# zoltanmaric/h264-fer

Hardware: AMD Instinct MI355X
Metric: macroblocks/sec encode (1080p full-search ME) + bit-exact bitstream vs ref (higher is better)
Workload: dtype u8; 1 GPU; 1080p IPPP encode, full-search +-16 ME (BASELINE configs[2]); content=textured, coded_size=1920x1072, streams_per_gpu=256, contexts_per_gpu=1, gop=30, qp=12, window=32, maxdiff=3, parallelism=1 x 256 independent closed-GOP streams

## Files before the change

h264-fer_amd/__init__.py:

```python
from .ferhip import (FerHip, FerHipError, Decoder, LiveDecoder, access_units, DeviceBuffer, Y4MReader, decode_streams, unescape_nal, lib_path,
                     load_library, mb_unit, cavlc_blocks, cavlc_parse_blocks, residual_mbs, RES_WRITE, RES_PARSE, mc_sub_mb_parts, MBU_QT, MBU_DEC4, MBU_DEC16, MBU_DECC, MBU_SKIP, TUNE_RESOLVE_WGS, TUNE_RESOLVE_GROUP, TUNE_SPECULATE, TUNE_OVERLAP_SORT, RC_CQP, RC_ABR, RC_QUALITY, QM_SSE, QM_SSIM,
                     QUALITY_RING, Quality, NAL_SLICE, NAL_IDR, NAL_AUTO, NAL_NONE, AU_PARAM_SETS, AU, frame_nal_blocks, frame_nal_blocks_raw,
                     NAL_UNIT, SPLIT_PREFIX, split_nal_blocks, split_nal_blocks_raw, FMT_I420, FMT_NV12, FMT_YUY2, FMT_UYVY, FMT_BGRA, FMT_RGBA, CSC_BT601, CSC_BT709, Pic, pic_table,
                     AU_AVCC, IN_ANNEXB, IN_AVCC, split_avcc_blocks_raw)
from .synth import gen_frame, gen_frames, crop_to_mb, pad_to_mb
from .shard import gops_of_rank, merge_gop_streams, split_nals
```

h264-fer_amd/csrc/fer_me.hip:

```cpp
#include <stdlib.h>
#include "fer_internal.h"
#include "fer_mvpred.h"

#define INF_M 1000000000

struct WList {
    int m;
    int xy;
};

__device__ __forceinline__ int pack_xy(int x, int y) { return (x & 0xffff) | (y << 16); }
__device__ __forceinline__ int unp_x(int xy) { return (int)(short)(xy & 0xffff); }
__device__ __forceinline__ int unp_y(int xy) { return xy >> 16; }

__device__ __forceinline__ void wl_insert(WList &L, int K, int lane, bool valid, int m, int xy)
{
    int thr = lane_bcast(L.m, K - 1);
    unsigned long long mask = __ballot(valid && m < thr);
    while (mask) {
        int src = __ffsll((long long)mask) - 1;
        mask &= mask - 1;
        int cm = lane_bcast(m, src), cxy = lane_bcast(xy, src);
        int pos = __popcll(__ballot(lane < K && L.m <= cm));
        if (pos < K) {
            int um = FER_DPP(L.m, DPP_WAVE_SHR1), uxy = FER_DPP(L.xy, DPP_WAVE_SHR1);
            if (lane > pos && lane < K) {
                L.m = um;
                L.xy = uxy;
            } else if (lane == pos) {
                L.m = cm;
                L.xy = cxy;
            }
        }
    }
}

#define WAVE_LDS_SYNC()                                    \
    do {                                                   \
        __builtin_amdgcn_fence(__ATOMIC_SEQ_CST, "wavefront"); \
        __builtin_amdgcn_wave_barrier();                   \
    } while (0)
__device__ __forceinline__ int lds_rank64(const unsigned *p, unsigned mine, int n4 = 16)
{
    const uint4 *q = (const uint4 *)p;
    int r = 0;
#pragma unroll 4
    for (int i = 0; i < n4; i++) {
        uint4 k = q[i];
        r += (int)(k.x < mine) + (int)(k.y < mine) + (int)(k.z < mine) + (int)(k.w < mine);
    }
    return r;
}

template <int NB, bool ORDERED, class RAW, class FIN, class ARR>
__device__ __forceinline__ bool select_topk_ex(const int (&v)[NB], int K, int lane, int *sel, WList &L, RAW raw, FIN fin, ARR arr)
{
    unsigned *A = (unsigned *)sel, *B = A + 64;
    int *Ci = sel + 128, *Di = sel + 192;
    const unsigned long long lt = (1ull << lane) - 1ull;
    int lmin = 0x7fffffff, lmax = -1, total = 0;
#pragma unroll
    for (int u = 0; u < NB; u++) {
        total += __popcll(__ballot(v[u] >= 0));
        lmin = (int)min((unsigned)lmin, (unsigned)v[u]);
        lmax = max(lmax, v[u]);
    }
    const int need = min(K, total);
    L.m = INF_M;
    L.xy = 0;
    if (need == 0) return true;
    int c = 65;
    if (!__any(lmax >= (1 << 26))) {
        B[lane] = 0xffffffffu;
        int T0 = 0x7fffffff;
        if (__popcll(__ballot(lmin != 0x7fffffff)) >= need) {
            int lo = 0, hi = (1 << 21) - 1;
            if (__popcll(__ballot(lmin <= hi)) >= need) {
                while (lo < hi) {
                    const int mid = (lo + hi) >> 1;
                    if (__popcll(__ballot(lmin <= mid)) >= need)
                        hi = mid;
                    else
                        lo = mid + 1;
                }
                T0 = lo;
            } else {
                T0 = 1 << 21;
            }
        }
        WAVE_LDS_SYNC();
        if (T0 < (1 << 21) && NB * 64 <= 2048) {
            int nsurv = 0;
#pragma unroll
            for (int u = 0; u < NB; u++) {
                const bool take = (unsigned)v[u] <= (unsigned)T0;
                const unsigned long long mk = __ballot(take);
                if (mk) {
                    const int slot = nsurv + (int)__builtin_amdgcn_mbcnt_hi((uint32_t)(mk >> 32), __builtin_amdgcn_mbcnt_lo((uint32_t)mk, 0u));
                    if (take && slot < 64) {
                        B[slot] = ((unsigned)v[u] << 11) | (unsigned)arr(u);
                        Ci[slot] = raw(u);
                    }
                    nsurv += __popcll(mk);
                }
            }
            WAVE_LDS_SYNC();
            c = nsurv;
        }
    }
    if (c <= 64) {
        WAVE_LDS_SYNC();
        const unsigned mine = B[lane];
        const int mypay = Ci[lane];
        const int rk = lds_rank64(B, mine, (__builtin_amdgcn_readfirstlane(c) + 3) >> 2);
        WAVE_LDS_SYNC();
        if (lane < c && rk < need) {
            A[rk] = mine >> 11;
            Di[rk] = mypay;
        }
        WAVE_LDS_SYNC();
        if (lane < need) {
            L.m = (int)A[lane];
            L.xy = fin(Di[lane]);
        }
        WAVE_LDS_SYNC();
        return true;
    }
    if (!ORDERED) return false;
    int *key = sel, *kxy = sel + 64, *key2 = sel + 128, *kxy2 = sel + 192;
    int lo = wave_min(lmin), hi;
    if (__popcll(__ballot(lmin != 0x7fffffff)) >= need)
        hi = wave_max(lmin != 0x7fffffff ? lmin : -1);
    else
        hi = wave_max(lmax);
    while (lo < hi) {
        int mid = lo + ((hi - lo) >> 1);
        int cnt = 0;
#pragma unroll
        for (int u = 0; u < NB; u++) cnt += __popcll(__ballot(v[u] >= 0 && v[u] <= mid));
        if (cnt >= need)
            hi = mid;
        else
            lo = mid + 1;
    }
    const int T = lo;
    int c_less = 0;
#pragma unroll
    for (int u = 0; u < NB; u++) c_less += __popcll(__ballot(v[u] >= 0 && v[u] < T));
    const int take_eq = need - c_less;
    int nsel = 0, eq_seen = 0;
    WAVE_LDS_SYNC();
#pragma unroll
    for (int u = 0; u < NB; u++) {
        bool ok = v[u] >= 0;
        bool eq = ok && v[u] == T;
        unsigned long long meq = __ballot(eq);
        bool take = (ok && v[u] < T) || (eq && eq_seen + __popcll(meq & lt) < take_eq);
        unsigned long long mt = __ballot(take);
        if (take) {
            int pos = nsel + __popcll(mt & lt);
            key[pos] = v[u];
            kxy[pos] = raw(u);
        }
        nsel += __popcll(mt);
        eq_seen += __popcll(meq);
    }
    WAVE_LDS_SYNC();
    int mk = lane < need ? key[lane] : INF_M, mxy = lane < need ? kxy[lane] : 0;
    int rank = 0;
    for (int i = 0; i < need; i++) {
        int ki = key[i];
        rank += (ki < mk) || (ki == mk && i < lane);
    }
    if (lane < need) {
        key2[rank] = mk;
        kxy2[rank] = mxy;
    }
    WAVE_LDS_SYNC();
    if (lane < need) {
        L.m = key2[lane];
        L.xy = fin(kxy2[lane]);
    }
    WAVE_LDS_SYNC();
    return true;
}
template <int NB, class RAW, class FIN>
__device__ __forceinline__ void select_topk(const int (&v)[NB], int K, int lane, int *sel, WList &L, RAW raw, FIN fin)
{
    select_topk_ex<NB, true>(v, K, lane, sel, L, raw, fin, [&](int u) { return u * 64 + lane; });
}

typedef unsigned short u16x2_t __attribute__((ext_vector_type(2)));
typedef short i16x2_t __attribute__((ext_vector_type(2)));
__device__ __forceinline__ uint32_t pk_sub16(uint32_t a, uint32_t b)
{
    return __builtin_bit_cast(uint32_t, (u16x2_t)(__builtin_bit_cast(u16x2_t, a) - __builtin_bit_cast(u16x2_t, b)));
}
__device__ __forceinline__ uint32_t pk_abs16(uint32_t a)
{
    i16x2_t x = __builtin_bit_cast(i16x2_t, a), z = {0, 0};
    return __builtin_bit_cast(uint32_t, __builtin_elementwise_max(x, (i16x2_t)(z - x)));
}
struct SuPk {
    uint32_t s01, s23, s4;
    uint32_t d01, d23, d4;
    uint32_t s12, s34;
    uint32_t e12, e34;
};
__device__ __forceinline__ SuPk su_pack(const int s[5])
{
    SuPk p;
    p.s01 = (uint32_t)s[0] | ((uint32_t)s[1] << 16);
    p.s23 = (uint32_t)s[2] | ((uint32_t)s[3] << 16);
    p.s4 = (uint32_t)s[4];
    p.d01 = (uint32_t)(s[0] - s[1]) << 16;
    p.d23 = (uint32_t)(s[0] - s[2]) | ((uint32_t)(s[0] - s[3]) << 16);
    p.d4 = (uint32_t)(s[0] - s[4]);
    p.s12 = (uint32_t)s[1] | ((uint32_t)s[2] << 16);
    p.s34 = (uint32_t)s[3] | ((uint32_t)s[4] << 16);
    p.e12 = (uint32_t)(s[0] - s[1]) | ((uint32_t)(s[0] - s[2]) << 16);
    p.e34 = (uint32_t)(s[0] - s[3]) | ((uint32_t)(s[0] - s[4]) << 16);
    return p;
}
__device__ __forceinline__ int feat_dist_w(uint32_t a, uint32_t b, uint32_t c, const SuPk &p)
{
    uint32_t t = __builtin_amdgcn_sad_u16(a, p.s01, 0);
    t = __builtin_amdgcn_sad_u16(b, p.s23, t);
    t = __builtin_amdgcn_sad_u16(c, p.s4, t);
    uint32_t kk = __builtin_amdgcn_perm(a, a, 0x01000100);
    t = __builtin_amdgcn_sad_u16(pk_sub16(kk, a), p.d01, t);
    t = __builtin_amdgcn_sad_u16(pk_sub16(kk, b), p.d23, t);
    t = __builtin_amdgcn_sad_u16(pk_sub16(kk, c) & 0xffffu, p.d4, t);
    return (int)t;
}
__device__ __forceinline__ int feat_dist_rec(const uint16_t *__restrict__ rec, const SuPk &p)
{
    const uint32_t *r = (const uint32_t *)rec;
    return feat_dist_w(r[0], r[1], r[2], p);
}
struct FeatRec {
    uint32_t a, b, c;
};
// ... 254 lines not shown
    su[1] = wave_sum(py > 3 ? 0 : v);
    su[2] = wave_sum(px > 3 ? 0 : v);
    su[3] = wave_sum((py & 3) > 1 ? 0 : v);
    su[4] = wave_sum((px & 3) > 1 ? 0 : v);
    if (lane < 5) d.suma[pidx * 5 + lane] = su[lane];
    if (d.basic) {
        if (lane == 0) {
            d.st3n[pidx] = 0;
            d.v0[pidx] = 0;
        }
        return;
    }
    const SuPk sp = su_pack(su);
    PP_MARK(0)

    WList L;
    L.m = INF_M;
    L.xy = 0;
    const int R = window / 2, n = 2 * R + 1;
    const int r2 = window / 16, n2w = 2 * r2 + 1, nloc = n2w * n2w * 16;
    const uint16_t *F0 = d.feat0 + (size_t)s * 6 * ysz;
    const int wb = (n * n + 63) >> 6;
    if ((WIN == 32 || WIN == 16) && !FER_DBGF(d, 3)) {
        constexpr int WCH = 3;
        constexpr int NN = (WIN ? WIN : 32) + 1;
        constexpr int NBc = WIN ? WIN : 32, RPB = 64 / NBc, NWB = (NN + RPB - 1) / RPB;
        constexpr int LB = LocalGeo<RRL>::NB;
        static_assert(LB <= 7, "ME_SEL_NB leaves room for 7 local batches");
        const int ix = lane % NBc, r0 = lane / NBc;
        const int rx = sx - R + ix;
        const bool xok = rx >= 0 && rx < W;
        const int wx = iabs(ix - R) + 4;
        const uint32_t colo = (uint32_t)iclamp(rx, 0, W - 1) * 12u, rowb = (uint32_t)W * 12u;
        auto fin = [&](int idx) {
            if (idx < wb * 64) return pack_xy((idx / n - R) * 4, (idx % n - R) * 4);
            int c = idx - wb * 64;
            int frac = c & 15, pos = c >> 4;
            return pack_xy((pos / n2w - r2) * 4 + (frac & 3), (pos % n2w - r2) * 4 + (frac >> 2));
        };
        uint32_t k0w[NWB];
#pragma unroll
        for (int b2 = 0; b2 < NWB; b2++) {
            const int ry = iclamp(sy - R + b2 * RPB + r0, 0, H - 1);
            k0w[b2] = *(const uint32_t *)((const char *)F0 + (colo + __umul24((uint32_t)ry, rowb)));
        }
        const uint32_t k0c = feat0_load(F0, W, H, sy - R + min(lane, NN - 1), sx + R).a;
        auto second_group = [&](int half) {
            if (half == 0) local_request<RRL>(ip, W, H, sx - RRL, sy - RRL, lane, ld, 1, 2);
        };
        local_metrics<RRL, decltype(second_group), true>(ip, W, H, sx - r2, sy - r2, sp, lane, (uint32_t *)wide_m, sel_lds, 0, 2, &ld, second_group);
        unsigned lminl = 0xffffffffu;
#pragma unroll
        for (int u = 0; u < LB; u++) lminl = min(lminl, (unsigned)sel_lds[u * 64 + lane]);
        int T = 0x7fffffff;
        if (__popcll(__ballot(lminl < (1u << 21))) >= 33) {
            int lo = 0, hi = (1 << 21) - 1;
            while (lo < hi) {
                const int mid = (lo + hi) >> 1;
                if (__popcll(__ballot(lminl <= (unsigned)mid)) >= 33)
                    hi = mid;
                else
                    lo = mid + 1;
            }
            T = lo;
        }
        int *surv = wide_m;
        int ns = 0;
        const uint32_t s0 = (uint32_t)su[0];
        bool done = false;
        if (T != 0x7fffffff) {
            static_assert((NBc / 2) % RPB == 0 && NN <= 64, "a batch stays on one side of the centre row");
            const int iy_lo = max(0, R - sy), iy_hi = min(NN - 1, H - 1 - (sy - R));
            const unsigned long long rowv = ((2ull << iy_hi) - 1ull) & ~((1ull << iy_lo) - 1ull);
            const unsigned long long colv = wave_ballot(xok);
            constexpr unsigned long long GRP = NBc == 64 ? ~0ull : (1ull << NBc) - 1ull;
            const uint32_t w5lo = 5u * (uint32_t)(wx + R - r0), w5hi = 5u * (uint32_t)(wx - R + r0);
            const int arr0 = ix * NN + r0;
#pragma unroll
            for (int b2 = 0; b2 < NWB; b2++) {
                unsigned long long valid = 0;
#pragma unroll
                for (int j = 0; j < RPB; j++)
                    if ((rowv >> (b2 * RPB + j)) & 1ull) valid |= GRP << (j * NBc);
                valid &= colv;
                const uint32_t w5 = b2 * RPB < R ? w5lo - 5u * (uint32_t)(b2 * RPB) : w5hi + 5u * (uint32_t)(b2 * RPB);
                const uint32_t lb = __umul24(w5, __builtin_amdgcn_sad_u16(k0w[b2] & 0xffffu, s0, 0u));
                const unsigned long long mk = wave_ballot(lb <= (uint32_t)T) & valid;
                if (mk) {
                    const int slot = ns + (int)__builtin_amdgcn_mbcnt_hi((uint32_t)(mk >> 32), __builtin_amdgcn_mbcnt_lo((uint32_t)mk, 0u));
                    if (wave_mask_bit(mk) && slot < 128) surv[slot] = arr0 + b2 * RPB;
                    ns += __popcll(mk);
                }
            }
            {
                const uint32_t lb = __umul24(5u * (uint32_t)(R + 4 + iabs(lane - R)), __builtin_amdgcn_sad_u16(k0c & 0xffffu, s0, 0u));
                const unsigned long long mk = sx + R < W ? wave_ballot(lb <= (uint32_t)T) & rowv : 0ull;
                if (mk) {
                    const int slot = ns + (int)__builtin_amdgcn_mbcnt_hi((uint32_t)(mk >> 32), __builtin_amdgcn_mbcnt_lo((uint32_t)mk, 0u));
                    if (wave_mask_bit(mk) && slot < 128) surv[slot] = (NN - 1) * NN + lane;
                    ns += __popcll(mk);
                }
            }
            WAVE_LDS_SYNC();
            if (ns <= 128) {
                int v[2 + LB], ar[2];
#pragma unroll
                for (int b2 = 0; b2 < 2; b2++) {
                    v[b2] = -1;
                    ar[b2] = 0;
                    if (b2 * 64 < ns) {
                        const int idx = b2 * 64 + lane;
                        const bool on = idx < ns;
                        const int ai = on ? surv[idx] : 0;
                        const int cix = ai / NN, ciy = ai - cix * NN;
                        const FeatRec f = feat0_load(F0, W, H, sy - R + ciy, sx - R + cix);
                        const int m = (int)__umul24((uint32_t)(iabs(cix - R) + iabs(ciy - R) + 4), (uint32_t)feat_dist_w(f.a, f.b, f.c, sp));
                        v[b2] = on ? m : -1;
                        ar[b2] = ai;
                    }
                }
#pragma unroll
                for (int u = 0; u < LB; u++) v[2 + u] = sel_lds[u * 64 + lane];
                WAVE_LDS_SYNC();
                auto arrv = [&](int u) { return u < 2 ? ar[u < 2 ? u : 0] : wb * 64 + (u - 2) * 64 + lane; };
                done = select_topk_ex<2 + LB, false>(v, 33, lane, wide_m + 128, L, arrv, fin, arrv);
            }
        }
        PP_MARK(1)
#ifdef FER_STATS
        if (lane == 0) {
            atomicAdd((unsigned long long *)&d.timing[48], 1ull);
            atomicAdd((unsigned long long *)&d.timing[49], done ? 0ull : 1ull);
            atomicAdd((unsigned long long *)&d.timing[50], (unsigned long long)ns);
            atomicAdd((unsigned long long *)&d.timing[51], T == 0x7fffffff ? 1ull : 0ull);
            atomicAdd((unsigned long long *)&d.timing[52], (unsigned long long)(T == 0x7fffffff ? 0 : T));
        }
#endif
        if (!done) {
            WAVE_LDS_SYNC();
            int vloc[LB];
#pragma unroll
            for (int u = 0; u < LB; u++) vloc[u] = sel_lds[u * 64 + lane];
            WAVE_LDS_SYNC();
            auto wide_load = [&](int iy0, FeatRec (&fr)[WCH]) {
#pragma unroll
                for (int q = 0; q < WCH; q++) {
                    int ry = iclamp(sy - R + iy0 + q * RPB + r0, 0, H - 1);
                    const uint32_t *r = (const uint32_t *)((const char *)F0 + (colo + __umul24((uint32_t)ry, rowb)));
                    fr[q].a = r[0];
                    fr[q].b = r[1];
                    fr[q].c = r[2];
                }
            };
            auto wide_eval = [&](int iy0, const FeatRec (&fr)[WCH]) {
#pragma unroll
                for (int q = 0; q < WCH; q++) {
                    const int iy = iy0 + q * RPB + r0;
                    const int ry = sy - R + iy;
                    const int m = (int)__umul24((uint32_t)(wx + iabs(iy - R)), (uint32_t)feat_dist_w(fr[q].a, fr[q].b, fr[q].c, sp));
                    const int bad = (xok && ry >= 0 && ry < H) ? 0 : -1;
                    wide_m[iy < n ? ix * n + iy : ME_WIDE_LDS - 1] = m | bad;
                }
            };
            {
                constexpr int STEP = RPB * WCH;
                FeatRec fa[WCH], fb[WCH];
                wide_load(0, fa);
                for (int iy0 = 0; iy0 < n; iy0 += 2 * STEP) {
                    if (iy0 + STEP < n) wide_load(iy0 + STEP, fb);
                    wide_eval(iy0, fa);
                    if (iy0 + STEP < n) {
                        if (iy0 + 2 * STEP < n) wide_load(iy0 + 2 * STEP, fa);
                        wide_eval(iy0 + STEP, fb);
                    }
                }
            }
            {
                const int iy = min(lane, n - 1);
// ... 858 lines not shown
                take = take && cls;
            }
            const int m = (r + 4) * D;
            const int side = kk0 > P.su[0] ? 1 : 0;
            const unsigned akey = ((unsigned)j << 21) | ((unsigned)(tx + 280) << 10) | (unsigned)(ty + 280);
            const int xy = pack_xy(tx * 4, ty * 4);
            cl_insert(L, lane, take, m, akey | ((unsigned)side << 20), xy);
            if (__any(take && j == 0)) cl_insert(L, lane, take && j == 0, m, akey | (1u << 20), xy);
            {
                int rr = (int)((1.0f + __fsqrt_rn((float)(2 * (k0 + 64) - 1))) * 0.5f);
                while (2 * rr * (rr - 1) + 1 > k0 + 64) rr--;
                while (2 * (rr + 1) * rr + 1 <= k0 + 64) rr++;
                done_r = rr - 1;
            }
            const int t33 = lane_bcast(L.m, 32);
            if (done_r >= rmax) break;
            if (t33 < INF_M && (long long)(done_r + 1 + 4) * dmin > (long long)t33) break;
        }
    }
    L2.m = L.m;
    L2.xy = L.xy;
}

__device__ __forceinline__ int stage2_list(const FerDev &d, int s, int gx, int gy, int lane, const ResPre &P, int genx, int geny,
                                           int *sel_lds, WList &L2)
{
    const int sx = gx * 8, sy = gy * 8;
    L2.m = INF_M;
    L2.xy = 0;
    if (d.basic || FER_DBGF(d, 32)) return 0;
    const uint32_t cfl = (uint32_t)lane_bcast(P.e2[0].y, 41);
    const bool rewalk = (cfl & 0x40000000u) != 0 && ((cfl >> 16) & 15u) == 0;
    if (P.n2raw > FER_ST2_CAP && d.zero_cnt[s] == 0 && !rewalk) {
        resolve_crowded(d, s, sx, sy, lane, P, genx, geny, L2);
    } else if (P.n2raw > FER_ST2_CAP) {
        const SuPk sp = su_pack(P.su);
        int jx;
        walk_buckets(d, s, P.su, sp, sx, sy, lane, (uint32_t *)sel_lds, 0x7fffffff, jx, [&](bool ok, int rank, int rel, int D, uint32_t, bool) {
            (void)rank;
            int tx = rel >> 16, ty = (int)(short)(rel & 0xffff);
            wl_insert(L2, 33, lane, ok, (iabs(tx - genx) + iabs(ty - geny) + 4) * D, pack_xy(tx * 4, ty * 4));
            return false;
        });
    } else {
        int m2[FER_ST2_CAP / 64];
#pragma unroll
        for (int u = 0; u < FER_ST2_CAP / 64; u++) {
            int cc = u * 64 + lane;
            int tx = P.e2[u].x >> 16, ty = (int)(short)(P.e2[u].x & 0xffff);
            m2[u] = (int)__umul24((uint32_t)(iabs(tx - genx) + iabs(ty - geny) + 4), (uint32_t)P.e2[u].y) | (cc < P.n2 ? 0 : -1);
        }
        auto raw2 = [&](int u) { return P.e2[u].x; };
        auto fin2 = [&](int e) { return pack_xy((e >> 16) * 4, (int)(short)(e & 0xffff) * 4); };
        select_topk<FER_ST2_CAP / 64>(m2, 33, lane, sel_lds, L2, raw2, fin2);
    }
    return __popcll(__ballot(lane < 33 && L2.m < 100000000));
}

template <int WIN>
__device__ __forceinline__ void resolve_stage23(const FerDev &d, int s, int gx, int gy, int lane, const ResPre &P, int mvpx, int mvpy,
                                                int *sel_lds, int &k2, int &xy2, int &k3, int &xy3)
{
    k2 = k3 = 0x7fffffff;
    xy2 = xy3 = 0;
    if (d.basic || FER_DBGF(d, 32)) return;
    WList L2;
    const int cnt2 = stage2_list(d, s, gx, gy, lane, P, mvpx >> 2, mvpy >> 2, sel_lds, L2);
    if (FER_DBGF(d, 256)) L2.xy = pack_xy(lane & 7, lane >> 3);
    int b2, b2xy;
    sad_keys<33>(L2, cnt2, lane, ip_stream(d, s), d.W, d.H, gx * 8, gy * 8, P.sb, mvpx, mvpy, b2, b2xy);
    wave_best(b2, b2xy, k2, xy2);
    int key = 0x7fffffff;
    if (lane < P.n3) key = ((P.c3s + iabs(P.c3x - mvpx) + iabs(P.c3y - mvpy)) << 6) | lane;
    wave_best(key, pack_xy(P.c3x, P.c3y), k3, xy3);
}

__device__ __forceinline__ ResNbr nbr_from_field(const FerDev &d, const int *vf, int gx, int gy, int lane)
{
    ResNbr N;
    nbr_avail(gx, gy, d.mbw * 2, N.vB, N.vC, N.vD, N.vC16);
    N.vA = gx > 0;
    const int xa = gx + (lane == 0 ? 0 : (lane == 1 ? 1 : (lane == 2 ? -1 : (lane == 3 ? 2 : -1)))), ya = lane == 4 ? gy : gy - 1;
    const bool val = lane == 0 ? N.vB : (lane == 1 ? N.vC : (lane == 2 ? N.vD : (lane == 3 ? N.vC16 : (lane == 4 && N.vA))));
    const int w = val ? vf[part_slot(d.mbw, xa, ya)] : 0;
    N.B = lane_bcast(w, 0);
    N.C = lane_bcast(w, 1);
    N.D = lane_bcast(w, 2);
    N.C16 = lane_bcast(w, 3);
    N.A = lane_bcast(w, 4);
    return N;
}

#ifndef SPEC_WAVES
#define SPEC_WAVES 7
#endif
template <int WIN>
__global__ __launch_bounds__(256) __attribute__((amdgpu_waves_per_eu(SPEC_WAVES, SPEC_WAVES))) void k_me_spec(FerDev d)
{
    __shared__ __attribute__((aligned(16))) uint32_t loc_all[4][LocalGeo<2>::HTAB + LocalGeo<2>::NB * 64];
    __shared__ int skipflag;
    static_assert(LocalGeo<2>::HTAB >= 256, "the selection's scratch fits the row sums");
    const int lane = threadIdx.x & 63;
    const int part = __builtin_amdgcn_readfirstlane(threadIdx.x >> 6);
    const int s = blockIdx.y;
    if (d.hdr[s * 4 + 3] != 0) return;
    const int mb = (int)xcd_swizzle(blockIdx.x, gridDim.x);
    const int mbx = mb % d.mbw, mby = mb / d.mbw;
// ... 260 lines not shown
        d.timing[7] = gw;
    }
#undef PR_MARK
    if (timeout && lane == 0) atomicOr(&d.status[s], FER_ERR_CHAIN_TIMEOUT);
    }
    if (lane == 0 && st_parts + st_skq > 0) {
        atomicAdd(&d.spec_stat[0], (unsigned long long)st_parts);
        atomicAdd(&d.spec_stat[1], (unsigned long long)st_hits);
        atomicAdd(&d.spec_stat[2], (unsigned long long)st_skq);
        atomicAdd(&d.spec_stat[3], (unsigned long long)st_skh);
    }
}

__global__ __launch_bounds__(64) void k_basic_stat(FerDev d)
{
    const int lane = threadIdx.x;
    const int s = blockIdx.y, mb = blockIdx.x;
    if (d.hdr[s * 4 + 3] != 0) return;
    if (d.mb_type[(size_t)s * d.nmb + mb] == FER_P_SKIP) return;
    const int W = d.W, H = d.H;
    const uint8_t *Y = d.curY + (size_t)s * d.ysz;
    const uint8_t *RY = d.refY + (size_t)s * d.ysz;
    const IPlanes ip = ip_stream(d, s);
    const int xp = (mb % d.mbw) << 4, yp = (mb / d.mbw) << 4;
    int src[4][4];
#pragma unroll
    for (int y = 0; y < 4; y++) {
        uint32_t v = *(const uint32_t *)(Y + (size_t)(yp + y) * W + xp);
#pragma unroll
        for (int k = 0; k < 4; k++) src[y][k] = (v >> (8 * k)) & 0xff;
    }
    const int R = d.window / 2, n = 2 * R + 1;
    int bsad = 0x7fffffff, bidx = 0x7fffffff;
    for (int c = lane; c < n * n; c += 64) {
        const int mvx = c / n - R, mvy = c % n - R;
        int sad = 0;
#pragma unroll
        for (int y = 0; y < 4; y++) {
            int p[4];
            mc_luma4(RY, ip, W, H, xp, yp, 0, y, mvx, mvy, p);
#pragma unroll
            for (int k = 0; k < 4; k++) sad += iabs(src[y][k] - p[k]);
        }
        if (sad < bsad) {
            bsad = sad;
            bidx = c;
        }
    }
    const int wsad = wave_min(bsad);
    const int widx = wave_min(bsad == wsad ? bidx : 0x7fffffff);
    if (lane == 0) atomicAdd(&d.stats[s * 5 + (widx == 0 ? 1 : 4)], 1);
}

void fer_launch_basic_stat(const FerDev &d, hipStream_t st)
{
    if (d.basic) hipLaunchKernelGGL(k_basic_stat, dim3(d.nmb, d.S), dim3(64), 0, st, d);
}

void fer_launch_me_pre(const FerDev &d, hipStream_t st)
{
    dim3 g(d.nmb * 4, d.S);
    if (d.window == 32)
        hipLaunchKernelGGL(k_me_pre<32>, g, dim3(64), 0, st, d);
    else if (d.window == 16)
        hipLaunchKernelGGL(k_me_pre<16>, g, dim3(64), 0, st, d);
    else
        hipLaunchKernelGGL(k_me_pre<0>, g, dim3(64), 0, st, d);
}

void fer_launch_me_walk(const FerDev &d, hipStream_t st)
{
    if (d.basic) return;
    hipLaunchKernelGGL(k_me_walk, dim3(d.nmb * 4, d.S), dim3(64), 0, st, d);
}

void fer_launch_me_spec(const FerDev &d, hipStream_t st)
{
    if (!d.speculate) return;
    dim3 g(d.nmb, d.S);
    if (d.window == 32)
        hipLaunchKernelGGL(k_me_spec<32>, g, dim3(256), 0, st, d);
    else if (d.window == 16)
        hipLaunchKernelGGL(k_me_spec<16>, g, dim3(256), 0, st, d);
    else
        hipLaunchKernelGGL(k_me_spec<0>, g, dim3(256), 0, st, d);
}

void fer_launch_me_resolve(const FerDev &d, hipStream_t st)
{
    const int gh = 2 * d.mbh;
    hipMemsetAsync(d.chain, 0, sizeof(int) * 8, st);
    const int cap = d.resolve_wgs;
    dim3 g(min(gh * d.S, max(cap, 1)));
    if (d.window == 32)
        hipLaunchKernelGGL(k_me_resolve<32>, g, dim3(64), 0, st, d);
    else if (d.window == 16)
        hipLaunchKernelGGL(k_me_resolve<16>, g, dim3(64), 0, st, d);
    else
        hipLaunchKernelGGL(k_me_resolve<0>, g, dim3(64), 0, st, d);
}
```

h264-fer_amd/csrc/fer_seam_host.h:

```cpp
#pragma once
#include "../../include/ferhip.h"
#include <stddef.h>
#include <stdint.h>

#define FER_SEAM_STREAM_MAX ((size_t)1 << 28)
#define FER_SEAM_BLOCKS_MAX ((size_t)1 << 30)
#define FER_SEAM_JOBS_MAX ((size_t)1 << 20)

static inline bool fer_seam_in(int32_t v, int32_t lo, int32_t hi) { return v >= lo && v <= hi; }

static inline bool fer_seam_block_ok(int32_t nC, int32_t max_num_coeff)
{
    if (max_num_coeff != 4 && max_num_coeff != 15 && max_num_coeff != 16) return false;
    if (nC < -1) return false;
    return nC != -1 || max_num_coeff == 4;
}

static inline int fer_seam_check_mb_unit(const ferhip_mb_job *jobs, const ferhip_mb_result *results, size_t n)
{
    if (!jobs || !results || n == 0) return FERHIP_E_ARG;
    for (size_t i = 0; i < n; i++) {
        const ferhip_mb_job &J = jobs[i];
        if (!fer_seam_in(J.op, FERHIP_MBU_QT, FERHIP_MBU_SKIP) || !fer_seam_in(J.cls, 0, 2) || !fer_seam_in(J.qp, 0, 51) ||
            !fer_seam_in(J.qpc, 0, 51) || !fer_seam_in(J.blk, 0, 15))
// ... 18 lines not shown
    if (!bits || !bit_pos || !nC || !max_num_coeff || !coef || !total_coeff || !bits_used || n == 0) return FERHIP_E_ARG;
    if (nbytes == 0 || nbytes > FER_SEAM_STREAM_MAX || n > FER_SEAM_BLOCKS_MAX) return FERHIP_E_ARG;
    for (size_t i = 0; i < n; i++)
        if (!fer_seam_block_ok(nC[i], max_num_coeff[i]) || bit_pos[i] >= (uint64_t)nbytes * 8) return FERHIP_E_ARG;
    return 0;
}

static inline int fer_seam_check_mc_parts(const uint8_t *ref_i420, int width, int height, const int32_t *desc, size_t n, const int32_t *predL,
                                          const int32_t *predCb, const int32_t *predCr)
{
    if (!ref_i420 || !desc || !predL || !predCb || !predCr || n == 0 || width <= 0 || height <= 0 || (width & 15) || (height & 15))
        return FERHIP_E_ARG;
    const int64_t nmb = (int64_t)(width >> 4) * (height >> 4);
    for (size_t i = 0; i < n; i++)
        if (desc[i * 5] < 0 || desc[i * 5] >= nmb || !fer_seam_in(desc[i * 5 + 1], 0, 3) || !fer_seam_in(desc[i * 5 + 2], 0, 3)) return FERHIP_E_ARG;
    return 0;
}

static inline bool fer_seam_levels16(const int32_t *v, size_t n)
{
    for (size_t i = 0; i < n; i++)
        if (v[i] < -32768 || v[i] > 32767) return false;
    return true;
}

static inline int fer_seam_check_residual_mbs(const ferhip_res_job *jobs, const ferhip_res_result *results, size_t n)
{
    if (!jobs || !results || n == 0 || n > FER_SEAM_JOBS_MAX) return FERHIP_E_ARG;
    for (size_t i = 0; i < n; i++) {
        const ferhip_res_job &J = jobs[i];
        if (!fer_seam_in(J.op, FERHIP_RES_WRITE, FERHIP_RES_PARSE) || !fer_seam_in(J.cls, 0, 2) || !fer_seam_in(J.cbp_luma, 0, 15) ||
            !fer_seam_in(J.cbp_chroma, 0, 2) || !fer_seam_in(J.avail, 0, 3))
            return FERHIP_E_ARG;
        if (J.cls == 1 && J.cbp_luma != 0 && J.cbp_luma != 15) return FERHIP_E_ARG;
        for (int k = 0; k < 2; k++) {
            if (!(J.avail & (1 << k))) continue;
            const ferhip_res_nb &N = J.nb[k];
            if (!fer_seam_in(N.p_skip, 0, 1) || !fer_seam_in(N.cbp_luma, 0, 15) || !fer_seam_in(N.cbp_chroma, 0, 2)) return FERHIP_E_ARG;
            for (int b = 0; b < 16; b++)
                if (!fer_seam_in(N.tc_luma[b], 0, 16)) return FERHIP_E_ARG;
            for (int b = 0; b < 8; b++)
                if (!fer_seam_in(N.tc_chroma[b >> 2][b & 3], 0, 16)) return FERHIP_E_ARG;
        }
        if (J.op == FERHIP_RES_PARSE) {
            if (J.nbytes == 0 || J.nbytes > FERHIP_RES_BITS_MAX || J.bit_pos >= J.nbytes * 8u) return FERHIP_E_ARG;
        } else if (!fer_seam_levels16(&J.lumaLevel[0][0], 256) || !fer_seam_levels16(J.dc16, 16) || !fer_seam_levels16(&J.ac16[0][0], 256) ||
                   !fer_seam_levels16(&J.cdc[0][0], 8) || !fer_seam_levels16(&J.cac[0][0][0], 128)) {
            return FERHIP_E_ARG;
        }
    }
    return 0;
}

static inline bool fer_seam_mb_addr_ok(int mb, int nmb) { return mb >= 0 && mb < nmb; }
```

h264-fer_amd/ferhip.py:

```python
import ctypes as C
import math
import os
from pathlib import Path

import numpy as np

NAL_SLICE, NAL_IDR, NAL_AUTO = 1, 5, 0
NAL_NONE = -1

BUF = dict(INTERP=1, FEAT=2, SORTPOS=3, KOLIKO=4, MBTYPE=5, MV=6, MVD=7, LEVELS=8, CBP=9, TC=10, I4MODE=11,
           CUR=12, REF=13, TIMING=14, ST2N=15, ST2=16, SPEC_STAT=17, MBSIZE=18,
           SUMA=19, ST3=20, ST3N=21, V0=22, SPEC_HDR=23, SPEC_L1=24, SPEC_L2=25)
TUNE_RESOLVE_WGS, TUNE_RESOLVE_GROUP, TUNE_SPECULATE, TUNE_OVERLAP_SORT = 1, 2, 3, 4
RC_CQP, RC_ABR, RC_QUALITY = 0, 1, 2
QM_SSE, QM_SSIM, QUALITY_RING = 1, 2, 64
AU_PARAM_SETS = 1
AU_AVCC = 4
IN_ANNEXB, IN_AVCC = 0, 1
_BUF_DTYPE = {1: np.uint8, 2: np.uint16, 3: np.uint32, 4: np.int32, 5: np.int32, 6: np.int16, 7: np.int16,
              8: np.int16, 9: np.uint8, 10: np.uint8, 11: np.uint8, 12: np.uint8, 13: np.uint8, 14: np.int64, 15: np.int32, 16: np.int32,
              17: np.uint64, 18: np.int32, 19: np.int32, 20: np.int32, 21: np.int32, 22: np.int32, 23: np.int32, 24: np.int32,
              25: np.int32}


# ... 683 lines not shown
    out = np.full(max(int(cap), 1), fill, np.uint8)
    units = np.zeros(max(int(units_cap), 1), NAL_UNIT)
    count = C.c_size_t(0)
    rc = lib.ferhip_split_nal_blocks(src.ctypes.data, stride, lens.ctypes.data, n, int(misalign), out.ctypes.data, int(cap),
                                     units.ctypes.data, int(units_cap), C.byref(count))
    return rc, out, units[: min(count.value, int(units_cap))], count.value


def split_avcc_blocks_raw(ranges, length_size, misalign=0, cap=None, units_cap=None, fill=0xA5):
    lib = load_library()
    n = len(ranges)
    lens = np.array([len(r) for r in ranges], np.uint32)
    stride = max(int(lens.max()) if n else 0, 1)
    src = np.zeros((n, stride), np.uint8)
    for k, r in enumerate(ranges):
        src[k, : len(r)] = np.frombuffer(bytes(r), np.uint8) if not isinstance(r, np.ndarray) else r
    if cap is None:
        cap = int(sum((int(m) // 3 + 1) * 16 + int(m) for m in lens))
    if units_cap is None:
        units_cap = int(sum(int(m) // 2 + 1 for m in lens))
    out = np.full(max(int(cap), 1), fill, np.uint8)
    units = np.zeros(max(int(units_cap), 1), NAL_UNIT)
    fault = np.full(max(n, 1), -1, np.int32)
    count = C.c_size_t(0)
    rc = lib.ferhip_split_avcc_blocks(src.ctypes.data, stride, lens.ctypes.data, n, int(misalign), int(length_size), out.ctypes.data,
                                      int(cap), units.ctypes.data, int(units_cap), C.byref(count), fault.ctypes.data)
    return rc, out, units[: min(count.value, int(units_cap))], count.value, fault[:n]


def split_nal_blocks(ranges, misalign=0):
    rc, out, units, _ = split_nal_blocks_raw(ranges, misalign)
    _chk(rc, "ferhip_split_nal_blocks")
    return [(int(u["range"]), int(u["nal_type"]), int(u["ref_idc"]), bytes(out[int(u["offset"]): int(u["offset"]) + int(u["bytes"])]))
            for u in units]


def frame_nal_blocks(payloads, nal_types):
    rc, out, idx = frame_nal_blocks_raw(payloads, nal_types)
    _chk(rc, "ferhip_frame_nal_blocks")
    return [bytes(out[int(e["offset"]): int(e["offset"]) + int(e["bytes"])]) for e in idx[:-1]]


def mc_sub_mb_parts(ref_i420, width, height, desc):
    lib = load_library()
    r = np.ascontiguousarray(ref_i420, np.uint8)
    d = np.ascontiguousarray(desc, np.int32).reshape(-1, 5)
    n = d.shape[0]
    pl, pb, pr = np.zeros((n, 4, 4), np.int32), np.zeros((n, 2, 2), np.int32), np.zeros((n, 2, 2), np.int32)
    lib.ferhip_mc_sub_mb_parts.argtypes = [C.c_void_p, C.c_int, C.c_int, C.c_void_p, C.c_size_t, C.c_void_p, C.c_void_p, C.c_void_p]
    _chk(lib.ferhip_mc_sub_mb_parts(r.ctypes.data, width, height, d.ctypes.data, n, pl.ctypes.data, pb.ctypes.data, pr.ctypes.data), "ferhip_mc_sub_mb_parts")
    return pl, pb, pr


def block_op(name, blocks, qp=0, flag=None):
    lib = load_library()
    a = np.ascontiguousarray(blocks, np.int32).reshape(-1, 16)
    out = np.empty_like(a)
    f = getattr(lib, "ferhip_" + name)
    if name == "transform_scan":
        rc = f(a.ctypes.data, out.ctypes.data, int(bool(flag)), a.shape[0])
    elif name == "transform_inverse_scan":
        rc = f(a.ctypes.data, out.ctypes.data, a.shape[0])
    else:
        rc = f(qp, a.ctypes.data, out.ctypes.data, a.shape[0])
    _chk(rc, "ferhip_" + name)
    return out


class Decoder:

    def __init__(self):
        self.lib = load_library()
        self.h = C.c_void_p()
        _chk(self.lib.ferhip_dec_create(C.byref(self.h)), "ferhip_dec_create")
        self.W = self.H = 0

    def nal(self, nal_unit_type, nal_ref_idc, rbsp):
        r = np.frombuffer(rbsp, np.uint8)
        got, W, H = C.c_int(), C.c_int(), C.c_int()
        pic = np.empty(self.W * self.H * 3 // 2, np.uint8) if nal_unit_type in (1, 5) else None
        _chk(self.lib.ferhip_dec_nal(self.h, nal_unit_type, nal_ref_idc, r.ctypes.data, len(rbsp),
                                     pic.ctypes.data if pic is not None else None, C.byref(got), C.byref(W), C.byref(H)),
             "ferhip_dec_nal")
        self.W, self.H = W.value, H.value
        return pic if got.value else None

    def close(self):
        if self.h:
            self.lib.ferhip_dec_destroy(self.h)
            self.h = C.c_void_p()

    def __del__(self):
        try:
            self.close()
        except Exception:
            pass


class LiveDecoder:

    def __init__(self, nstreams, width, height, max_pictures=1):
        self.lib = load_library()
        self.S, self.W, self.H, self.P = nstreams, width, height, max_pictures
        self.fsz = width * height * 3 // 2
        self.cfsz = self.fsz
        self.win, self.layout = (0, 0, width, height), None
# ... 214 lines not shown
```

include/ferhip.h:

```cpp
#ifndef FERHIP_H
#define FERHIP_H
#include <stddef.h>
#include <stdint.h>

#ifdef __cplusplus
extern "C" {
#endif

#define FERHIP_E_ARG -1
#define FERHIP_E_HIP -2
#define FERHIP_E_STATE -3
#define FERHIP_E_UNSUP -4
#define FERHIP_E_DEVICE -5

#define FERHIP_NAL_SLICE 1
#define FERHIP_NAL_IDR 5
#define FERHIP_NAL_AUTO 0
#define FERHIP_NAL_NONE -1

typedef struct ferhip_ctx ferhip_ctx;

typedef struct {
    int qp;
    int basic;
// ... 204 lines not shown
int ferhip_forward_residual(int qP, const int32_t *in, int32_t *out, int keep_dc, size_t nblocks);
int ferhip_inverse_residual(int qP, const int32_t *in, int32_t *out, int keep_dc, size_t nblocks);
int ferhip_forward_dc_luma_intra(int qP, const int32_t *in, int32_t *out, size_t nblocks);
int ferhip_inverse_dc_luma_intra(int qP, const int32_t *in, int32_t *out, size_t nblocks);
int ferhip_forward_dc_chroma(int qP, const int32_t *in, int32_t *out, size_t nblocks);
int ferhip_inverse_dc_chroma(int qP, const int32_t *in, int32_t *out, size_t nblocks);
int ferhip_transform_scan(const int32_t *in, int32_t *out, int intra16x16_ac, size_t nblocks);
int ferhip_transform_inverse_scan(const int32_t *in, int32_t *out, size_t nblocks);

#define FERHIP_MBU_QT 0
#define FERHIP_MBU_DEC4 1
#define FERHIP_MBU_DEC16 2
#define FERHIP_MBU_DECC 3
#define FERHIP_MBU_SKIP 4
typedef struct {
    int32_t op, cls , qp , qpc , reconstruct, blk;
    int32_t srcY[256], srcCb[64], srcCr[64];
    int32_t predY[256], predCb[64], predCr[64];
    int32_t lumaLevel[16][16], dc16[16], ac16[16][16], cdc[2][4], cac[2][4][16];
} ferhip_mb_job;
typedef struct {
    int32_t lumaLevel[16][16], dc16[16], ac16[16][16], cdc[2][4], cac[2][4][16];
    int32_t recY[256], recCb[64], recCr[64];
} ferhip_mb_result;
int ferhip_mb_unit(const ferhip_mb_job *jobs, ferhip_mb_result *results, size_t njobs);
int ferhip_cavlc_blocks(const int32_t *coef, const int32_t *nC, const int32_t *max_num_coeff, size_t nblocks, uint8_t *bits,
                        uint32_t *nbits, int32_t *total_coeff);
int ferhip_cavlc_parse_blocks(const uint8_t *bits, size_t nbytes, const uint64_t *bit_pos, const int32_t *nC,
                              const int32_t *max_num_coeff, size_t nblocks, int32_t *coef, int32_t *total_coeff,
                              uint32_t *bits_used);
#define FERHIP_RES_WRITE 0
#define FERHIP_RES_PARSE 1
#define FERHIP_RES_BITS_MAX 2048
typedef struct {
    int32_t p_skip, cbp_luma, cbp_chroma, tc_luma[16], tc_chroma[2][4];
} ferhip_res_nb;
typedef struct {
    int32_t op, cls , cbp_luma, cbp_chroma;
    int32_t avail;
    ferhip_res_nb nb[2];
    int32_t lumaLevel[16][16], dc16[16], ac16[16][16], cdc[2][4], cac[2][4][16];
    uint32_t bit_pos, nbytes;
    uint8_t bits[FERHIP_RES_BITS_MAX];
} ferhip_res_job;
typedef struct {
    int32_t nbits;
    int32_t tc_luma[16], tc_chroma[2][4];
    int32_t lumaLevel[16][16], dc16[16], ac16[16][16], cdc[2][4], cac[2][4][16];
    uint8_t bits[FERHIP_RES_BITS_MAX];
} ferhip_res_result;
int ferhip_residual_mbs(const ferhip_res_job *jobs, ferhip_res_result *results, size_t njobs);
int ferhip_mc_sub_mb_parts(const uint8_t *ref_i420, int width, int height, const int32_t *desc, size_t n, int32_t *predL,
                           int32_t *predCb, int32_t *predCr);

#ifdef __cplusplus
}
#endif
#endif
```

Before: 22.38 million macroblocks/s.

## Replace ballot binary search with bitwise threshold probe and reuse wide-stage threshold

Replaces the per-wave binary search for the top-K selection threshold with a radix-style bit-by-bit probe that first tests a small range (bit 12 or 16), so typical small metrics need fewer ballot rounds. The wide-candidate stage now hands its already computed threshold to the follow-up selection, which skips the search when that threshold still admits enough lanes and refines only if too many survivors appear. A host-callable test kernel and Python binding for the selection routine are added as well. The change cuts scalar ballot iterations in ME candidate selection, at the cost of more code paths and a possible extra gather pass.

```diff
diff --git a/h264-fer_amd/__init__.py b/h264-fer_amd/__init__.py
--- a/h264-fer_amd/__init__.py
+++ b/h264-fer_amd/__init__.py
@@ -2,6 +2,6 @@
                      load_library, mb_unit, cavlc_blocks, cavlc_parse_blocks, residual_mbs, RES_WRITE, RES_PARSE, mc_sub_mb_parts, MBU_QT, MBU_DEC4, MBU_DEC16, MBU_DECC, MBU_SKIP, TUNE_RESOLVE_WGS, TUNE_RESOLVE_GROUP, TUNE_SPECULATE, TUNE_OVERLAP_SORT, RC_CQP, RC_ABR, RC_QUALITY, QM_SSE, QM_SSIM,
                      QUALITY_RING, Quality, NAL_SLICE, NAL_IDR, NAL_AUTO, NAL_NONE, AU_PARAM_SETS, AU, frame_nal_blocks, frame_nal_blocks_raw,
                      NAL_UNIT, SPLIT_PREFIX, split_nal_blocks, split_nal_blocks_raw, FMT_I420, FMT_NV12, FMT_YUY2, FMT_UYVY, FMT_BGRA, FMT_RGBA, CSC_BT601, CSC_BT709, Pic, pic_table,
-                     AU_AVCC, IN_ANNEXB, IN_AVCC, split_avcc_blocks_raw)
+                     AU_AVCC, IN_ANNEXB, IN_AVCC, split_avcc_blocks_raw, select_kat, SEL_WIDE, SEL_REFINED, SEL_GENERAL, SEL_REFUSED)
 from .synth import gen_frame, gen_frames, crop_to_mb, pad_to_mb
 from .shard import gops_of_rank, merge_gop_streams, split_nals
diff --git a/h264-fer_amd/csrc/fer_me.hip b/h264-fer_amd/csrc/fer_me.hip
--- a/h264-fer_amd/csrc/fer_me.hip
+++ b/h264-fer_amd/csrc/fer_me.hip
@@ -1,6 +1,8 @@
 #include <stdlib.h>
 #include "fer_internal.h"
+#include "fer_ctx.h"
 #include "fer_mvpred.h"
+#include "fer_seam_host.h"
 
 #define INF_M 1000000000
 
@@ -52,8 +54,53 @@
     return r;
 }
 
-template <int NB, bool ORDERED, class RAW, class FIN, class ARR>
-__device__ __forceinline__ bool select_topk_ex(const int (&v)[NB], int K, int lane, int *sel, WList &L, RAW raw, FIN fin, ARR arr)
+#define SEL_T_NONE 0x7fffffff
+#define SEL_T_BIG (1 << 21)
+template <int E0>
+__device__ __forceinline__ int lane_min_threshold(unsigned lmin, int need, int hint = SEL_T_NONE)
+{
+    static_assert(E0 == 12 || E0 == 16, "the first probe");
+    auto lanes_below = [&](unsigned p) {
+        int c = __builtin_popcountll(__builtin_amdgcn_ballot_w64(lmin < p));
+        asm("" : "+s"(c));
+        return c;
+    };
+    auto below = [&](unsigned p) { return hint < (int)p || lanes_below(p) >= need; };
+    int top = E0;
+    if (!below(1u << E0)) {
+        if (E0 < 16 && below(1u << 16)) {
+            top = 16;
+        } else {
+            if (lanes_below(0x7fffffffu) < need) return SEL_T_NONE;
+            if (!below(1u << 21)) return SEL_T_BIG;
+            top = 21;
+        }
+    }
+    unsigned res = 0;
+    auto step = [&](int b) {
+        const unsigned p = res + (1u << b);
+        if (lanes_below(p) < need) res = p;
+    };
+    if (top > 16) {
+#pragma unroll
+        for (int b = 20; b >= 16; b--) step(b);
+    }
+    if (top > 12) {
+#pragma unroll
+        for (int b = 15; b >= 12; b--) step(b);
+    }
+#pragma unroll
+    for (int b = 11; b >= 0; b--) step(b);
+    return (int)res;
+}
+
+#define SEL_ROUTE_WIDE 0
+#define SEL_ROUTE_REFINED 1
+#define SEL_ROUTE_GENERAL 2
+#define SEL_ROUTE_REFUSED 3
+template <int NB, bool ORDERED, int E0 = 12, class RAW, class FIN, class ARR>
+__device__ __forceinline__ bool select_topk_ex(const int (&v)[NB], int K, int lane, int *sel, WList &L, RAW raw, FIN fin, ARR arr, int given = -1,
+                                               int *route = nullptr)
 {
     unsigned *A = (unsigned *)sel, *B = A + 64;
     int *Ci = sel + 128, *Di = sel + 192;
@@ -68,32 +115,19 @@
     const int need = min(K, total);
     L.m = INF_M;
     L.xy = 0;
+    if (route) *route = SEL_ROUTE_WIDE;
     if (need == 0) return true;
     int c = 65;
     if (!__any(lmax >= (1 << 26))) {
         B[lane] = 0xffffffffu;
-        int T0 = 0x7fffffff;
-        if (__popcll(__ballot(lmin != 0x7fffffff)) >= need) {
-            int lo = 0, hi = (1 << 21) - 1;
-            if (__popcll(__ballot(lmin <= hi)) >= need) {
-                while (lo < hi) {
-                    const int mid = (lo + hi) >> 1;
-                    if (__popcll(__ballot(lmin <= mid)) >= need)
-                        hi = mid;
-                    else
-                        lo = mid + 1;
-                }
-                T0 = lo;
-            } else {
-                T0 = 1 << 21;
-            }
-        }
+        const bool loose = given >= 0 && given < (1 << 21) && __builtin_popcountll(__builtin_amdgcn_ballot_w64((unsigned)lmin <= (unsigned)given)) >= need;
+        int T0 = loose ? given : lane_min_threshold<E0>((unsigned)lmin, need);
         WAVE_LDS_SYNC();
-        if (T0 < (1 << 21) && NB * 64 <= 2048) {
+        auto gather = [&](int T) {
             int nsurv = 0;
 #pragma unroll
             for (int u = 0; u < NB; u++) {
-                const bool take = (unsigned)v[u] <= (unsigned)T0;
+                const bool take = (unsigned)v[u] <= (unsigned)T;
                 const unsigned long long mk = __ballot(take);
                 if (mk) {
                     const int slot = nsurv + (int)__builtin_amdgcn_mbcnt_hi((uint32_t)(mk >> 32), __builtin_amdgcn_mbcnt_lo((uint32_t)mk, 0u));
@@ -105,7 +139,17 @@
                 }
             }
             WAVE_LDS_SYNC();
-            c = nsurv;
+            return nsurv;
+        };
+        if (T0 < (1 << 21) && NB * 64 <= 2048) {
+            c = gather(T0);
+            if (loose && c > 64) {
+                T0 = lane_min_threshold<E0>((unsigned)lmin, need, T0);
+                B[lane] = 0xffffffffu;
+                WAVE_LDS_SYNC();
+                c = gather(T0);
+                if (route) *route = SEL_ROUTE_REFINED;
+            }
         }
     }
     if (c <= 64) {
@@ -126,6 +170,7 @@
         WAVE_LDS_SYNC();
         return true;
     }
+    if (route) *route = ORDERED ? SEL_ROUTE_GENERAL : SEL_ROUTE_REFUSED;
     if (!ORDERED) return false;
     int *key = sel, *kxy = sel + 64, *key2 = sel + 128, *kxy2 = sel + 192;
     int lo = wave_min(lmin), hi;
@@ -184,10 +229,10 @@
     WAVE_LDS_SYNC();
     return true;
 }
-template <int NB, class RAW, class FIN>
+template <int NB, int E0 = 12, class RAW, class FIN>
 __device__ __forceinline__ void select_topk(const int (&v)[NB], int K, int lane, int *sel, WList &L, RAW raw, FIN fin)
 {
-    select_topk_ex<NB, true>(v, K, lane, sel, L, raw, fin, [&](int u) { return u * 64 + lane; });
+    select_topk_ex<NB, true, E0>(v, K, lane, sel, L, raw, fin, [&](int u) { return u * 64 + lane; });
 }
 
 typedef unsigned short u16x2_t __attribute__((ext_vector_type(2)));
@@ -548,18 +593,8 @@
         unsigned lminl = 0xffffffffu;
 #pragma unroll
         for (int u = 0; u < LB; u++) lminl = min(lminl, (unsigned)sel_lds[u * 64 + lane]);
-        int T = 0x7fffffff;
-        if (__popcll(__ballot(lminl < (1u << 21))) >= 33) {
-            int lo = 0, hi = (1 << 21) - 1;
-            while (lo < hi) {
-                const int mid = (lo + hi) >> 1;
-                if (__popcll(__ballot(lminl <= (unsigned)mid)) >= 33)
-                    hi = mid;
-                else
-                    lo = mid + 1;
-            }
-            T = lo;
-        }
+        int T = lane_min_threshold<12>(lminl, 33);
+        if (T >= SEL_T_BIG) T = 0x7fffffff;
         int *surv = wide_m;
         int ns = 0;
         const uint32_t s0 = (uint32_t)su[0];
@@ -619,7 +654,7 @@
                 for (int u = 0; u < LB; u++) v[2 + u] = sel_lds[u * 64 + lane];
                 WAVE_LDS_SYNC();
                 auto arrv = [&](int u) { return u < 2 ? ar[u < 2 ? u : 0] : wb * 64 + (u - 2) * 64 + lane; };
-                done = select_topk_ex<2 + LB, false>(v, 33, lane, wide_m + 128, L, arrv, fin, arrv);
+                done = select_topk_ex<2 + LB, false>(v, 33, lane, wide_m + 128, L, arrv, fin, arrv, T);
             }
         }
         PP_MARK(1)
@@ -1584,7 +1619,7 @@
         }
         auto raw2 = [&](int u) { return P.e2[u].x; };
         auto fin2 = [&](int e) { return pack_xy((e >> 16) * 4, (int)(short)(e & 0xffff) * 4); };
-        select_topk<FER_ST2_CAP / 64>(m2, 33, lane, sel_lds, L2, raw2, fin2);
+        select_topk<FER_ST2_CAP / 64, 16>(m2, 33, lane, sel_lds, L2, raw2, fin2);
     }
     return __popcll(__ballot(lane < 33 && L2.m < 100000000));
 }
@@ -1951,6 +1986,62 @@
     if (lane == 0) atomicAdd(&d.stats[s * 5 + (widx == 0 ? 1 : 4)], 1);
 }
 
+template <int NB, bool ORDERED>
+__global__ __launch_bounds__(64) void k_select_kat(const int32_t *__restrict__ metrics, const int32_t *__restrict__ arrival,
+                                                   const int32_t *__restrict__ threshold, int K, int n, int32_t *__restrict__ list_m,
+                                                   int32_t *__restrict__ list_pay, int32_t *__restrict__ route)
+{
+    __shared__ __attribute__((aligned(16))) int sel[256];
+    const int lane = threadIdx.x;
+    for (int row = blockIdx.x; row < n; row += gridDim.x) {
+        const size_t base = (size_t)row * (NB * 64);
+        int v[NB], ar[NB];
+#pragma unroll
+        for (int u = 0; u < NB; u++) {
+            v[u] = metrics[base + u * 64 + lane];
+            ar[u] = ORDERED ? u * 64 + lane : arrival[base + u * 64 + lane];
+        }
+        const int given = threshold ? __builtin_amdgcn_readfirstlane(threshold[row]) : -1;
+        WList L;
+        int rt;
+        auto arrv = [&](int u) { return ar[u]; };
+        select_topk_ex<NB, ORDERED, NB == 6 ? 16 : 12>(v, K, lane, sel, L, arrv, [](int a) { return a; }, arrv, given, &rt);
+        list_m[(size_t)row * 64 + lane] = L.m;
+        list_pay[(size_t)row * 64 + lane] = L.xy;
+        if (lane == 0) route[row] = rt;
+        WAVE_LDS_SYNC();
+    }
+}
+
+extern "C" int ferhip_select_kat(const int32_t *metrics, size_t nrows, int nb, int k, const int32_t *arrival, const int32_t *threshold,
+                                 int32_t *list_metric, int32_t *list_payload, int32_t *route)
+{
+    if (fer_seam_check_select(metrics, nrows, nb, k, arrival, threshold, list_metric, list_payload, route)) return FERHIP_E_ARG;
+    const size_t per = (size_t)nb * 64;
+    DevBuf<int32_t> dm, da, dt, dlm, dlp, dr;
+    if (dm.reserve(nrows * per) || (arrival && da.reserve(nrows * per)) || (threshold && dt.reserve(nrows)) || dlm.reserve(nrows * 64) ||
+        dlp.reserve(nrows * 64) || dr.reserve(nrows))
+        return FERHIP_E_HIP;
+    CK(hipMemcpy(dm, metrics, nrows * per * 4, hipMemcpyHostToDevice));
+    if (arrival) CK(hipMemcpy(da, arrival, nrows * per * 4, hipMemcpyHostToDevice));
+    if (threshold) CK(hipMemcpy(dt, threshold, nrows * 4, hipMemcpyHostToDevice));
+    const dim3 g((unsigned)(nrows < 2048 ? nrows : 2048)), b(64);
+    const int n = (int)nrows;
+    if (nb == 6)
+        hipLaunchKernelGGL((k_select_kat<6, true>), g, b, 0, 0, dm.p, da.p, dt.p, k, n, dlm.p, dlp.p, dr.p);
+    else if (nb == 7)
+        hipLaunchKernelGGL((k_select_kat<7, true>), g, b, 0, 0, dm.p, da.p, dt.p, k, n, dlm.p, dlp.p, dr.p);
+    else if (nb == 9)
+        hipLaunchKernelGGL((k_select_kat<9, false>), g, b, 0, 0, dm.p, da.p, dt.p, k, n, dlm.p, dlp.p, dr.p);
+    else
+        hipLaunchKernelGGL((k_select_kat<ME_SEL_NB, true>), g, b, 0, 0, dm.p, da.p, dt.p, k, n, dlm.p, dlp.p, dr.p);
+    CK(hipGetLastError());
+    CK(hipMemcpy(list_metric, dlm, nrows * 64 * 4, hipMemcpyDeviceToHost));
+    CK(hipMemcpy(list_payload, dlp, nrows * 64 * 4, hipMemcpyDeviceToHost));
+    CK(hipMemcpy(route, dr, nrows * 4, hipMemcpyDeviceToHost));
+    return 0;
+}
+
 void fer_launch_basic_stat(const FerDev &d, hipStream_t st)
 {
     if (d.basic) hipLaunchKernelGGL(k_basic_stat, dim3(d.nmb, d.S), dim3(64), 0, st, d);
diff --git a/h264-fer_amd/csrc/fer_seam_host.h b/h264-fer_amd/csrc/fer_seam_host.h
--- a/h264-fer_amd/csrc/fer_seam_host.h
+++ b/h264-fer_amd/csrc/fer_seam_host.h
@@ -94,4 +94,19 @@
     return 0;
 }
 
+#define FER_SEAM_SELECT_ROWS_MAX ((size_t)1 << 16)
+static inline int fer_seam_check_select(const int32_t *metrics, size_t nrows, int nb, int k, const int32_t *arrival, const int32_t *threshold,
+                                        const int32_t *list_metric, const int32_t *list_payload, const int32_t *route)
+{
+    if (!metrics || !list_metric || !list_payload || !route || nrows == 0 || nrows > FER_SEAM_SELECT_ROWS_MAX) return FERHIP_E_ARG;
+    if (nb != 6 && nb != 7 && nb != 9 && nb != 25) return FERHIP_E_ARG;
+    if ((nb == 9) != (arrival != NULL) || k < 1 || k > 64) return FERHIP_E_ARG;
+    const size_t tot = nrows * (size_t)nb * 64;
+    for (size_t i = 0; i < tot; i++)
+        if (metrics[i] < -1 || metrics[i] >= (1 << 29) || (arrival && !fer_seam_in(arrival[i], 0, 2047))) return FERHIP_E_ARG;
+    for (size_t i = 0; threshold && i < nrows; i++)
+        if (threshold[i] < -1 || threshold[i] >= (1 << 29)) return FERHIP_E_ARG;
+    return 0;
+}
+
 static inline bool fer_seam_mb_addr_ok(int mb, int nmb) { return mb >= 0 && mb < nmb; }
diff --git a/h264-fer_amd/ferhip.py b/h264-fer_amd/ferhip.py
--- a/h264-fer_amd/ferhip.py
+++ b/h264-fer_amd/ferhip.py
@@ -759,6 +759,24 @@
     return pl, pb, pr
 
 
+SEL_WIDE, SEL_REFINED, SEL_GENERAL, SEL_REFUSED = 0, 1, 2, 3
+
+
+def select_kat(metrics, k, arrival=None, threshold=None):
+    lib = load_library()
+    m = np.ascontiguousarray(metrics, np.int32)
+    n, nb = m.shape[0], m.shape[1]
+    assert m.shape == (n, nb, 64)
+    a = None if arrival is None else np.ascontiguousarray(arrival, np.int32)
+    assert a is None or a.shape == m.shape
+    t = None if threshold is None else np.ascontiguousarray(threshold, np.int32).reshape(n)
+    lm, lp, rt = np.zeros((n, 64), np.int32), np.zeros((n, 64), np.int32), np.zeros(n, np.int32)
+    lib.ferhip_select_kat.argtypes = [C.c_void_p, C.c_size_t, C.c_int, C.c_int] + [C.c_void_p] * 5
+    _chk(lib.ferhip_select_kat(m.ctypes.data, n, nb, int(k), None if a is None else a.ctypes.data, None if t is None else t.ctypes.data,
+                               lm.ctypes.data, lp.ctypes.data, rt.ctypes.data), "ferhip_select_kat")
+    return lm, lp, rt
+
+
 def block_op(name, blocks, qp=0, flag=None):
     lib = load_library()
     a = np.ascontiguousarray(blocks, np.int32).reshape(-1, 16)
diff --git a/include/ferhip.h b/include/ferhip.h
--- a/include/ferhip.h
+++ b/include/ferhip.h
@@ -280,6 +280,12 @@
 int ferhip_residual_mbs(const ferhip_res_job *jobs, ferhip_res_result *results, size_t njobs);
 int ferhip_mc_sub_mb_parts(const uint8_t *ref_i420, int width, int height, const int32_t *desc, size_t n, int32_t *predL,
                            int32_t *predCb, int32_t *predCr);
+#define FERHIP_SEL_WIDE 0
+#define FERHIP_SEL_REFINED 1
+#define FERHIP_SEL_GENERAL 2
+#define FERHIP_SEL_REFUSED 3
+int ferhip_select_kat(const int32_t *metrics, size_t nrows, int nb, int k, const int32_t *arrival, const int32_t *threshold,
+                      int32_t *list_metric, int32_t *list_payload, int32_t *route);
 
 #ifdef __cplusplus
 }
```

After: 22.84 million macroblocks/s, median of 6. 1.02x the previous value.
